# sara-nl/saraGAN

Measured on AMD Instinct MI355X. Metric: 3D volumes/sec/node (G+D step) at 128x128x32, higher is better.
Workload: dtype bf16

## Files before the change

### saragan_amd/csrc/common.h

```cpp
#pragma once
#include <hip/hip_runtime.h>
#include <stdint.h>
#include <mutex>
#include "../../include/saragan_hip.h"

typedef __bf16 bf16_t;
typedef float f32x4 __attribute__((ext_vector_type(4)));
typedef float f32x16 __attribute__((ext_vector_type(16)));
typedef __bf16 bf16x8 __attribute__((ext_vector_type(8)));
typedef __bf16 bf16x4 __attribute__((ext_vector_type(4)));
typedef short s16x4 __attribute__((ext_vector_type(4)));
typedef uint32_t u32x4 __attribute__((ext_vector_type(4)));

#define SG_STORE16_GUARD(v) asm volatile("s_nop 1" ::"v"(v))
typedef uint32_t u32x2 __attribute__((ext_vector_type(2)));

#define SG_LAUNCH_CHECK()                          \
  do {                                             \
    hipError_t e__ = hipGetLastError();            \
    if (e__ != hipSuccess) return (int)e__;        \
  } while (0)

static inline hipStream_t sg_st(sg_stream_t s) { return (hipStream_t)s; }

struct sg_config {
  int fwd_lds, fwd_tg;
  int fwd_v1, fwd_no_pw, fwd_no_dense;
  int fwd_no_v3, fwd_no_v3s, fwd_no_v4, fwd_no_v5, fwd_no_ksplit;
  int fwd3p_16;
  int fwd3s_16;
  int fwd_no_3p;
  int fwd3_gx, fwd3_no_lean;
  int fwd4_gx, fwd4_no_lean, fwd4_no_wres;
  int wgrad_v1, wgrad_no_v3, wgrad_no_lean;
  int wgrad_no_w16;
  int wgrad3l_min_cols;
  int wgrad3l_16;
  int wgrad3l_reuse;
  int wgrad_v1_blocks;
  int dbg_flags;
  int no_small;
  int deterministic;
  int gemm_ks_model;
  int gemm_k333_maxvox;
  int no_gemm;
};
const sg_config& sg_cfg();

bool sg_gemm_conv_eligible(const sg_conv_shape* s, sg_dtype dt);
size_t sg_gemm_conv_workspace(const sg_conv_shape* s, sg_dtype dt);
int sg_gemm_conv_fwd(const void* x, const void* wp, void* y, const sg_conv_shape* s, const float* bias, int act, float slope,
                     const uint32_t* mask_bits, float mask_slope, uint32_t* sign_out, void* workspace, size_t workspace_bytes,
                     hipStream_t st, bool* used);

bool sg_small_eligible(const sg_conv_shape* s);
bool sg_small_wgrad_eligible(const sg_conv_shape* s);
size_t sg_small_tail_bytes(const sg_conv_shape* s);
size_t sg_small_wgrad_workspace(const sg_conv_shape* s);
int sg_small_pack(const float* w, float coef, int flip, void* tail, const sg_conv_shape* s, sg_dtype dt, hipStream_t st);
int sg_small_fwd(const void* x, const void* tail, void* y, const sg_conv_shape* s, const float* bias, int act, float slope,
                 int pixel_norm, float eps, float* pn_scale, const uint32_t* mask_bits, float mask_slope, uint32_t* sign_out,
                 sg_dtype dt, hipStream_t st);
int sg_small_wgrad(const void* x, const void* dy, float* dw, float* dbias, float coef, void* workspace, size_t workspace_bytes,
                   const sg_conv_shape* s, sg_dtype dt, hipStream_t st);

#define SG_ALLOW_160K_LDS(kern)                                                                                  \
  do {                                                                                                           \
    static std::once_flag once__;                                                                                \
    static hipError_t err__ = hipSuccess;                                                                        \
    std::call_once(once__, [&] {                                                                                 \
      err__ = hipFuncSetAttribute((const void*)(kern), hipFuncAttributeMaxDynamicSharedMemorySize, 160 * 1024);  \
    });                                                                                                          \
    if (err__ != hipSuccess) return (int)err__;                                                                  \
  } while (0)
static inline size_t sg_esize(sg_dtype dt) { return dt == SG_BF16 ? 2 : 4; }
static inline bool sg_aligned16(const void* p) { return (((uintptr_t)p) & 15) == 0; }

__device__ __forceinline__ void philox4x32_10(uint32_t c0, uint32_t c1, uint32_t c2, uint32_t c3, uint32_t k0,
                                              uint32_t k1, uint32_t out[4]) {
#pragma unroll
  for (int rnd = 0; rnd < 10; ++rnd) {
    const uint32_t hi0 = __umulhi(0xD2511F53u, c0), lo0 = 0xD2511F53u * c0;
    const uint32_t hi1 = __umulhi(0xCD9E8D57u, c2), lo1 = 0xCD9E8D57u * c2;
    const uint32_t n0 = hi1 ^ c1 ^ k0, n1 = lo1, n2 = hi0 ^ c3 ^ k1, n3 = lo0;
    c0 = n0; c1 = n1; c2 = n2; c3 = n3;
    k0 += 0x9E3779B9u; k1 += 0xBB67AE85u;
  }
  out[0] = c0; out[1] = c1; out[2] = c2; out[3] = c3;
}

struct sg_fastdiv {
  uint32_t d, m;
};
static inline __host__ __device__ sg_fastdiv sg_make_fastdiv(uint32_t d) {
  sg_fastdiv f;
  f.d = d;
  f.m = d <= 1 ? 0u : (uint32_t)((0x100000000ull + d - 1) / d);
  return f;
}
__device__ __forceinline__ uint32_t sg_div(uint32_t x, sg_fastdiv f) {
  return f.d <= 1 ? x : __umulhi(x, f.m);
}

template <typename T>
struct sg_traits;
template <>
struct sg_traits<float> {
  static constexpr int CH = 8;
  __device__ static __forceinline__ float to_f(float v) { return v; }
  __device__ static __forceinline__ float from_f(float v) { return v; }
};
template <>
struct sg_traits<bf16_t> {
  static constexpr int CH = 16;
  __device__ static __forceinline__ float to_f(bf16_t v) { return (float)v; }
  __device__ static __forceinline__ bf16_t from_f(float v) { return (bf16_t)v; }
};

template <typename T>
__device__ __forceinline__ f32x16 sg_mfma_chunk(u32x4 a, u32x4 b, f32x16 c);
template <>
__device__ __forceinline__ f32x16 sg_mfma_chunk<bf16_t>(u32x4 a, u32x4 b, f32x16 c) {
// ... 200 lines not shown
```

### saragan_amd/csrc/prof.hip

```cpp
#include "prof.h"
#include <mutex>
#include <vector>
#include <string.h>
#include <stdlib.h>
#include <atomic>

namespace {
struct Rec { int kind; sg_conv_shape shape; int dtype; hipEvent_t e0, e1; bool ok; const char* name; };
std::mutex g_mu;
bool g_on = false;
bool g_filter = false;
int g_fkind = 0;
sg_conv_shape g_fshape;
std::vector<Rec> g_recs;
const char* kVersion = "saragan_hip 0.4 (gfx950)";
}

bool sg_prof_on() { return g_on; }
thread_local const char* sg_tls_kernel = "";

namespace {
std::atomic<const sg_config*> g_cfg{nullptr};
int env_int(const char* name, int dflt) {
  const char* v = getenv(name);
  return v && *v ? atoi(v) : dflt;
}
const sg_config* read_config() {
  sg_config* c = new sg_config;
  c->fwd_lds = env_int("SG_FWD_LDS", 80 * 1024);
  c->fwd_tg = env_int("SG_FWD_TG", 0);
  c->fwd_v1 = env_int("SG_FWD_V1", 0);
  c->fwd_no_pw = env_int("SG_FWD_NO_PW", 0);
  c->fwd_no_dense = env_int("SG_FWD_NO_DENSE", 0);
  c->fwd_no_v3 = env_int("SG_FWD_NO_V3", 0);
  c->fwd_no_v3s = env_int("SG_FWD_NO_V3S", 0);
  c->wgrad_no_lean = env_int("SG_WGRAD_NO_LEAN", 0);
  c->wgrad_no_w16 = env_int("SG_WGRAD_NO_W16", 0);
  c->wgrad3l_16 = env_int("SG_WGRAD3L_16", 0);
  c->wgrad3l_reuse = env_int("SG_WGRAD3L_REUSE", 1);
  c->wgrad3l_min_cols = env_int("SG_WGRAD3L_MIN_COLS", 0);
  c->wgrad_v1_blocks = env_int("SG_WGRAD_V1_BLOCKS", 0);
  c->fwd_no_v4 = env_int("SG_FWD_NO_V4", 0);
  c->fwd_no_v5 = env_int("SG_FWD_NO_V5", 0);
  c->fwd_no_ksplit = env_int("SG_FWD_NO_KSPLIT", 0);
  c->fwd_no_3p = env_int("SG_FWD_NO_3P", 0);
  c->fwd3p_16 = env_int("SG_FWD3P_16", 1);
  c->fwd3s_16 = env_int("SG_FWD3S_16", 1);
  c->fwd3_gx = env_int("SG_FWD3_GX", 0);
  c->fwd3_no_lean = env_int("SG_FWD3_NO_LEAN", 0);
  c->fwd4_gx = env_int("SG_FWD4_GX", 0);
  c->fwd4_no_lean = env_int("SG_FWD4_NO_LEAN", 0);
  c->fwd4_no_wres = env_int("SG_FWD4_NO_WRES", 0);
  c->wgrad_v1 = env_int("SG_WGRAD_V1", 0);
  c->wgrad_no_v3 = env_int("SG_WGRAD_NO_V3", 0);
  c->dbg_flags = env_int("SG_DBG_FLAGS", 0);
  c->no_small = env_int("SG_NO_SMALL", 0);
  c->deterministic = env_int("SG_DETERMINISTIC", 0);
  c->no_gemm = env_int("SG_NO_GEMM", 0);
  c->gemm_ks_model = env_int("SG_GEMM_KS_MODEL", 0);
  c->gemm_k333_maxvox = env_int("SG_GEMM_K333_MAXVOX", 8192);
  return c;
}
}

const sg_config& sg_cfg() {
  const sg_config* c = g_cfg.load(std::memory_order_acquire);
  if (c == nullptr) {
    std::lock_guard<std::mutex> lk(g_mu);
    c = g_cfg.load(std::memory_order_acquire);
    if (c == nullptr) {
      c = read_config();
      g_cfg.store(c, std::memory_order_release);
    }
  }
  return *c;
}

extern "C" int sg_config_reload(void) {
  std::lock_guard<std::mutex> lk(g_mu);
  g_cfg.store(read_config(), std::memory_order_release);
  return SG_OK;
}

void sg_prof_begin(int kind, const sg_conv_shape* s, sg_dtype dt, hipStream_t st, int* slot) {
  std::lock_guard<std::mutex> lk(g_mu);
  if (g_filter && (kind != g_fkind || memcmp(s, &g_fshape, sizeof(sg_conv_shape)) != 0)) { *slot = -1; return; }
  Rec r; r.kind = kind; r.shape = *s; r.dtype = (int)dt; r.ok = false; r.name = "";
  if (hipEventCreate(&r.e0) != hipSuccess) { *slot = -1; return; }
  if (hipEventCreate(&r.e1) != hipSuccess) { (void)hipEventDestroy(r.e0); *slot = -1; return; }
  (void)hipEventRecord(r.e0, st);
  g_recs.push_back(r);
  *slot = (int)g_recs.size() - 1;
}

void sg_prof_end(int slot, hipStream_t st) {
  std::lock_guard<std::mutex> lk(g_mu);
  bool ok = slot >= 0;
  int idx = ok ? slot : -1 - slot;
  if (idx < 0 || idx >= (int)g_recs.size()) return;
  (void)hipEventRecord(g_recs[idx].e1, st);
  g_recs[idx].ok = ok;
}

void sg_prof_name(int slot, const char* name) {
  std::lock_guard<std::mutex> lk(g_mu);
  if (slot >= 0 && slot < (int)g_recs.size()) g_recs[slot].name = name;
}

extern "C" const char* sg_version(void) { return kVersion; }

extern "C" const char* sg_error_string(int code) {
  switch (code) {
    case SG_OK: return "ok";
    case SG_EINVAL: return "invalid argument (shape, null pointer or unsupported combination)";
    case SG_EWORKSPACE: return "workspace too small";
    case SG_EALIGN: return "pointer not 16-byte aligned";
    case SG_EUNSUPPORTED: return "no kernel covers this request";
    default: break;
  }
  if (code > 0) return hipGetErrorString((hipError_t)code);
  return "unknown error";
}

extern "C" int sg_prof_enable(int on) {
// ... 51 lines not shown
```

### saragan_amd/csrc/wgrad.hip

```cpp
#include "common.h"
#include "prof.h"
#include <stdlib.h>
#include <type_traits>

struct WgradArgs {
  const void* x;
  const void* dy;
  float* dwt;
  sg_tile_geom g;
  sg_tile_geom gy;
  int cin, cout, taps, kh, kw, tap0, taps_blk;
  int ciT, coT;
  int rs;
  int xbytes, ybytes;
  int ntiles;
  sg_fastdiv fnp;
  int vec_x, vec_y;
  int plane_rows;
  float* dbias;
  int64_t slab, bslab;
  int nslab;
  int dbg_flags;
  unsigned long long* dbg;
  const uint32_t* dy_mask;
// ... 1546 lines not shown
  *used = false;
  const bool w16 = KD == 3 && KH == 3 && KW == 3 && s->w == 16 && (s->h % 8) == 0 && (s->d % 2) == 0 && !a.dy_mask &&
                   !sg_cfg().wgrad_no_lean && !sg_cfg().wgrad_no_w16;
  a.g = sg_make_geom(s, 256, true, 2, w16 ? 8 : 4);
  const sg_tile_geom& g = a.g;
  if (g.TW != (w16 ? 16 : 32) || g.TN != 1 || g.TD * g.TH * g.TW != 256) return SG_OK;
  if (g.HD != 2 && g.HD != 4) return SG_OK;
  if (g.TD != 2 || g.TH != (w16 ? 8 : 4)) return SG_OK;
  if (g.HH > 127 || g.HW > 127) return SG_OK;
  if ((s->cin % 8) || (s->cout % 8)) return SG_OK;
  if ((int64_t)g.TN * s->d * s->h * s->w * (int64_t)(s->cin > s->cout ? s->cin : s->cout) >= (1ll << 31)) return SG_OK;
  const int ncol = g.nTn * g.nTh * g.nTw;
  const int pairs = a.ciT * a.coT;
  int gx = (256 / pairs) / 8 * 8;
  if (gx < 8) gx = 8;
  while (gx > 8 && ncol < 2 * gx && (gx - 8) * pairs >= (w16 ? 128 : 64)) gx -= 8;
  const int min_cols = sg_cfg().wgrad3l_min_cols > 0 ? sg_cfg().wgrad3l_min_cols : 2;
  if (ncol < (2 * gx < min_cols ? 2 * gx : min_cols) || g.nTd < 2) return SG_OK;
  a.gy = a.g;
  a.ntiles = ncol * g.nTd;
  a.rs = 64;
  a.plane_rows = (g.HH * g.HW + 15) & ~15;
  if (a.plane_rows / 16 > 16) return SG_OK;
  a.xbytes = g.HD * a.plane_rows * 64;
  a.ybytes = 256 * 64;
  size_t lds = 2ull * (a.xbytes + a.ybytes);
  if (lds > 160 * 1024) return SG_OK;
  a.tap0 = 0; a.taps_blk = a.taps;
  a.nslab = 2 * gx;
  const bool lean = KD == 3 && KH == 3 && KW == 3 && g.HH == 6 && g.HW == 34 && g.HD == 4 && a.plane_rows == 208 &&
                    s->w % 32 == 0 && !sg_cfg().wgrad_no_lean && (!g.ups || ((s->d | s->h | s->w) & 1) == 0);
  const bool lean16 = w16 && g.HH == 10 && g.HW == 18 && g.HD == 4 && (!g.ups || ((s->d | s->h | s->w) & 1) == 0);
  if (w16 && !lean16) return SG_OK;
  if (lean16 || lean) a.nslab = gx;
  if (lean) lds += 12288;
  const bool m16 = sg_cfg().wgrad3l_16 != 0;
  const bool ru = sg_cfg().wgrad3l_reuse != 0;
#define SG_LAUNCH_WGRAD3L_1(UPS_, DYM_, TW_, M16_, RU_, NAME_)                                                        \
  do {                                                                                                               \
    auto kern = conv_wgrad3l_kernel<UPS_, DYM_, TW_, M16_, RU_>;                                                     \
    SG_ALLOW_160K_LDS(kern);                                                                                         \
    SG_KNAME(NAME_);                                                                                                 \
    hipLaunchKernelGGL(kern, dim3((unsigned)gx, (unsigned)pairs), dim3(512), lds, st, a);                            \
  } while (0)
#define SG_LAUNCH_WGRAD3L(UPS_, DYM_, TW_, NAME_)                                                                     \
  do {                                                                                                               \
    if (m16 && ru) SG_LAUNCH_WGRAD3L_1(UPS_, DYM_, TW_, true, true, NAME_);                                          \
    else if (m16) SG_LAUNCH_WGRAD3L_1(UPS_, DYM_, TW_, true, false, NAME_);                                          \
    else if (ru) SG_LAUNCH_WGRAD3L_1(UPS_, DYM_, TW_, false, true, NAME_);                                           \
    else SG_LAUNCH_WGRAD3L_1(UPS_, DYM_, TW_, false, false, NAME_);                                                  \
  } while (0)
  if (lean16) {
    lds = 2ull * (4 * 208 * 64 + 256 * 64) + 12288;
    if (g.ups) SG_LAUNCH_WGRAD3L(true, false, 16, "conv_wgrad3l<ups,w16>");
    else SG_LAUNCH_WGRAD3L(false, false, 16, "conv_wgrad3l<w16>");
  } else if (a.dy_mask) {
    if (!lean || g.ups || ((s->d | s->h | s->w) & 1)) return SG_OK;
    SG_LAUNCH_WGRAD3L(false, true, 32, "conv_wgrad3l<dy gather>");
  } else if (lean && g.ups) {
    SG_LAUNCH_WGRAD3L(true, false, 32, "conv_wgrad3l<ups>");
  } else if (lean) {
    SG_LAUNCH_WGRAD3L(false, false, 32, "conv_wgrad3l");
#undef SG_LAUNCH_WGRAD3L
#undef SG_LAUNCH_WGRAD3L_1
  } else {
    auto kern = conv_wgrad3_kernel<KD, KH, KW>;
    SG_ALLOW_160K_LDS(kern);
    SG_KNAME("conv_wgrad3<%d,%d,%d>", KD, KH, KW);
    hipLaunchKernelGGL(kern, dim3((unsigned)gx, (unsigned)pairs), dim3(512), lds, st, a);
  }
  SG_LAUNCH_CHECK();
  *used = true;
  return SG_OK;
}

struct WgradPlanesArgs {
  const void* x;
  const void* dy;
  float* dwt;
  float* dbias;
  int cin, cout, ciT, coT;
  int ntiles;
  int64_t slab, bslab;
};

template <int HW_>
__device__ __forceinline__ void conv_wgrad_planes_body(const WgradPlanesArgs& a) {
  extern __shared__ __attribute__((aligned(16))) char smem[];
  constexpr int H = HW_, W = HW_, P = 128 / (H * W), RP = (H + 2) * (W + 2);
  constexpr int XROWS = P * RP, NPX = (XROWS * 4 + 255) / 256, NPY = 2, PPT = NPX + NPY;
  constexpr int XB = NPX * 4096, YB = 128 * 64, BUF = XB + YB;
  constexpr uint32_t DEAD = 0x80000000u;
  const int tid = threadIdx.x, lane = tid & 63;
  const int wave = __builtin_amdgcn_readfirstlane(tid >> 6);
  const int ci_t = blockIdx.y / a.coT, co_t = blockIdx.y % a.coT;
  const int cin = a.cin, cout = a.cout;
  uint32_t vx[NPX], vy[NPY];
#pragma unroll
  for (int k = 0; k < NPX; ++k) {
    const int it = tid + 256 * k;
    const int row = it >> 2, sub = it & 3;
    const int p = row / RP, rr = row - p * RP;
    const int hh = rr / (W + 2), hw = rr - hh * (W + 2);
    const bool in = row < XROWS && hh >= 1 && hh <= H && hw >= 1 && hw <= W;
    vx[k] = in ? (uint32_t)((((p * H + hh - 1) * W + hw - 1) * cin + ci_t * 32 + sub * 8) * 2) : DEAD;
  }
#pragma unroll
  for (int k = 0; k < NPY; ++k) {
    const int it = tid + 256 * k;
    vy[k] = (uint32_t)(((it >> 2) * cout + co_t * 32 + (it & 3) * 8) * 2);
  }
  const __amdgpu_buffer_rsrc_t rx = __builtin_amdgcn_make_buffer_rsrc(const_cast<void*>(a.x), 0, (int)((int64_t)a.ntiles * 128 * cin * 2), 0x00020000);
  const __amdgpu_buffer_rsrc_t ry = __builtin_amdgcn_make_buffer_rsrc(const_cast<void*>(a.dy), 0, (int)((int64_t)a.ntiles * 128 * cout * 2), 0x00020000);
  auto stage = [&](int t, int b) __attribute__((always_inline)) {
    const bool ok = t < a.ntiles;
    const uint32_t sx = ok ? (uint32_t)t * (uint32_t)(128 * cin * 2) : 0u, sy = ok ? (uint32_t)t * (uint32_t)(128 * cout * 2) : 0u;
    char* xb = smem + b * BUF;
#pragma unroll
    for (int k = 0; k < NPX; ++k)
      __builtin_amdgcn_raw_ptr_buffer_load_lds(rx, (lds_ptr_t)(xb + (tid + 256 * k) * 16 - lane * 16), 16, ok ? vx[k] : DEAD, sx, 0, 0);
#pragma unroll
    for (int k = 0; k < NPY; ++k)
      __builtin_amdgcn_raw_ptr_buffer_load_lds(ry, (lds_ptr_t)(xb + XB + (tid + 256 * k) * 16 - lane * 16), 16, ok ? vy[k] : DEAD, sy, 0, 0);
  };
  const int i16 = lane & 15, q16 = lane >> 4;
  const int colb = (16 * (q16 & 1) + 4 * (i16 & 3)) * 2;
  const int kb = 8 * (q16 >> 1) + (i16 >> 2);
  int xr[2], yr[2];
#pragma unroll
  for (int j = 0; j < 2; ++j) {
    const int m = kb + 4 * j;
    xr[j] = ((m / W + (wave < 3 ? wave : 0)) * (W + 2) + m % W) * 64 + colb;
    yr[j] = XB + m * 64 + colb;
  }
  const bool ones = wave == 3 && a.dbias != nullptr && ci_t == 0;
  f32x16 acc[3];
#pragma unroll
  for (int j = 0; j < 3; ++j)
#pragma unroll
    for (int i = 0; i < 16; ++i) acc[j][i] = 0.f;
  const u32x4 one8 = {0x3F803F80u, 0x3F803F80u, 0x3F803F80u, 0x3F803F80u};

  typedef s16x4 __attribute__((address_space(3))) * lds_s16x4_p;
  const int t0 = blockIdx.x, G = gridDim.x;
  stage(t0, 0);
  stage(t0 + G, 1);
  int b = 0;
  for (int t = t0; t < a.ntiles; t += G) {
    const int b2 = b >= 1 ? b - 1 : 2;
    stage(t + 2 * G, b2);
    asm volatile("s_waitcnt vmcnt(%0)" ::"n"(2 * PPT) : "memory");
    __syncthreads();
    const char* base = smem + b * BUF;
    if (wave < 3 || ones) {
#pragma unroll
      for (int ks = 0; ks < 8; ++ks) {
        const int xoff = H == 8 ? ((ks >> 2) * RP + (ks & 3) * 2 * (W + 2)) * 64 : ks * RP * 64;
        const s16x4 b0 = __builtin_amdgcn_ds_read_tr16_b64_v4i16((lds_s16x4_p)(base + yr[0] + ks * 1024));
        const s16x4 b1 = __builtin_amdgcn_ds_read_tr16_b64_v4i16((lds_s16x4_p)(base + yr[1] + ks * 1024));
        u32x4 bf;
        bf[0] = __builtin_bit_cast(u32x2, b0)[0]; bf[1] = __builtin_bit_cast(u32x2, b0)[1];
        bf[2] = __builtin_bit_cast(u32x2, b1)[0]; bf[3] = __builtin_bit_cast(u32x2, b1)[1];
        if (wave < 3) {
#pragma unroll
          for (int kw = 0; kw < 3; ++kw) {
            const s16x4 a0 = __builtin_amdgcn_ds_read_tr16_b64_v4i16((lds_s16x4_p)(base + xr[0] + xoff + kw * 64));
            const s16x4 a1 = __builtin_amdgcn_ds_read_tr16_b64_v4i16((lds_s16x4_p)(base + xr[1] + xoff + kw * 64));
            u32x4 af;
            af[0] = __builtin_bit_cast(u32x2, a0)[0]; af[1] = __builtin_bit_cast(u32x2, a0)[1];
            af[2] = __builtin_bit_cast(u32x2, a1)[0]; af[3] = __builtin_bit_cast(u32x2, a1)[1];
            acc[kw] = __builtin_amdgcn_mfma_f32_32x32x16_bf16(__builtin_bit_cast(bf16x8, af), __builtin_bit_cast(bf16x8, bf), acc[kw], 0, 0, 0);
          }
        } else {
          acc[0] = __builtin_amdgcn_mfma_f32_32x32x16_bf16(__builtin_bit_cast(bf16x8, one8), __builtin_bit_cast(bf16x8, bf), acc[0], 0, 0, 0);
        }
      }
    }
    __syncthreads();
    b = b == 2 ? 0 : b + 1;
  }
  asm volatile("s_waitcnt vmcnt(0)" ::: "memory");
  const int r = lane & 31, hh = lane >> 5;
  const bool slab = a.slab != 0;
  if (wave < 3) {
#pragma unroll
    for (int kw = 0; kw < 3; ++kw) {
      float* dst = a.dwt + (int64_t)blockIdx.x * a.slab + ((((int64_t)(wave * 3 + kw) * a.ciT + ci_t) * a.coT + co_t) << 10);
#pragma unroll
      for (int i = 0; i < 16; ++i) {
        const int row = (i & 3) + 8 * (i >> 2) + 4 * hh;
        sg_wg_out(dst + row * 32 + r, acc[kw][i], slab);
      }
    }
  } else if (ones && hh == 0) {
    sg_wg_out(a.dbias + (int64_t)blockIdx.x * a.bslab + co_t * 32 + r, acc[0][0], slab);
  }
}

__global__ __launch_bounds__(256, 2) void conv_wgrad_planes8_kernel(WgradPlanesArgs a) { conv_wgrad_planes_body<8>(a); }
__global__ __launch_bounds__(256, 2) void conv_wgrad_planes4_kernel(WgradPlanesArgs a) { conv_wgrad_planes_body<4>(a); }

static bool wgrad_planes_eligible(const sg_conv_shape* s) {
  if (s->kd != 1 || s->kh != 3 || s->kw != 3 || s->upsample_in || s->h != s->w || (s->h != 4 && s->h != 8)) return false;
  if ((s->cin % 32) || (s->cout % 32)) return false;
  const int P = 128 / (s->h * s->w);
  const int64_t planes = (int64_t)s->n * s->d;
  if (planes % P) return false;
  const int64_t vox = planes * s->h * s->w;
  return vox * (s->cin > s->cout ? s->cin : s->cout) * 2 < (1ll << 31);
}

static int launch_wgrad_planes(WgradArgs& a, const sg_conv_shape* s, hipStream_t st, bool* used) {
  *used = false;
  if (!wgrad_planes_eligible(s)) return SG_OK;
  WgradPlanesArgs p;
  p.x = a.x; p.dy = a.dy; p.dwt = a.dwt; p.dbias = a.dbias; p.cin = s->cin; p.cout = s->cout; p.ciT = a.ciT; p.coT = a.coT;
  p.ntiles = (int)((int64_t)s->n * s->d * s->h * s->w / 128);
  p.slab = a.slab; p.bslab = a.bslab;
  const int pairs = a.ciT * a.coT;
  int gx = sg_cdiv(512, pairs);
  if (gx > 16) gx = 16;
  if (gx > p.ntiles) gx = p.ntiles;
  a.nslab = gx;
  if (s->h == 8) {
    auto kern = conv_wgrad_planes8_kernel;
    SG_ALLOW_160K_LDS(kern);
    SG_KNAME("conv_wgrad_planes<8>");
    constexpr int XB = ((2 * 100 * 4 + 255) / 256) * 4096;
    hipLaunchKernelGGL(kern, dim3((unsigned)gx, (unsigned)pairs), dim3(256), 3 * (size_t)(XB + 8192), st, p);
  } else {
    auto kern = conv_wgrad_planes4_kernel;
    SG_ALLOW_160K_LDS(kern);
    SG_KNAME("conv_wgrad_planes<4>");
    constexpr int XB = ((8 * 36 * 4 + 255) / 256) * 4096;
    hipLaunchKernelGGL(kern, dim3((unsigned)gx, (unsigned)pairs), dim3(256), 3 * (size_t)(XB + 8192), st, p);
  }
  SG_LAUNCH_CHECK();
  *used = true;
  return SG_OK;
}

static size_t wgrad_tile_bytes(const sg_conv_shape* s) {
  const size_t need = (size_t)(s->kd * s->kh * s->kw) * sg_cdiv(s->cin, 32) * sg_cdiv(s->cout, 32) * 4096;
  const bool pointwise = s->kd * s->kh * s->kw == 1 && (s->cin <= 4 || s->cout <= 4);
  const size_t pw = pointwise ? (size_t)PW_WGRAD_MAX_BLOCKS * 5 * (size_t)(s->cin > s->cout ? s->cin : s->cout) * sizeof(float) : 0;
  return ((need > pw ? need : pw) + 255) & ~(size_t)255;
}

extern "C" int sg_conv3d_wgrad(const void* x, const void* dy, float* dw, float coef, void* workspace,
                               size_t workspace_bytes, const sg_conv_shape* s, sg_dtype dt, sg_stream_t st) {
  return sg_conv3d_wgrad_bias(x, dy, dw, nullptr, coef, workspace, workspace_bytes, s, dt, st);
}

static int wgrad_bias_impl(const void* x, const void* dy, float* dw, float* dbias, float coef, void* workspace,
                           size_t workspace_bytes, const sg_conv_shape* s, sg_dtype dt, sg_stream_t st, void* pw_dx,
                           const float* pw_wmat, const void* dy_mask = nullptr, float dy_mask_slope = 0.f, float dy_gain = 1.f,
                           unsigned flags = 0) {
  const int accumulate = (flags & SG_WGRAD_ACCUMULATE) ? 1 : 0;
  const bool clean_ws = (flags & SG_WGRAD_CLEAN_WORKSPACE) != 0;
  if (!conv_shape_ok_w(s) || !x || !dy || !dw || !workspace) return SG_EINVAL;
  if (!sg_aligned16(x) || !sg_aligned16(dy) || !sg_aligned16(workspace)) return SG_EALIGN;
  if (dy_mask && (dt != SG_BF16 || s->kd != 3 || s->kh != 3 || s->kw != 3 || s->upsample_in || (s->cout % 32) ||
                  sg_cfg().wgrad_v1 || sg_cfg().wgrad_no_v3 || !sg_is_pow2f(dy_gain)))
    return SG_EUNSUPPORTED;
  const size_t need = sg_conv3d_wgrad_workspace(s, dt);
  if (workspace_bytes < need) return SG_EWORKSPACE;
  hipStream_t hs = sg_st(st);
  sg_prof_scope prof(1, s, dt, hs);
  {
    const int taps1 = s->kd * s->kh * s->kw;
    const int cs = s->cin < s->cout ? s->cin : s->cout, cb = s->cin < s->cout ? s->cout : s->cin;
    const int E = dt == SG_BF16 ? 8 : 4;
    if (taps1 == 1 && cs <= 4 && !s->upsample_in && cb % E == 0 && cb / E <= 256 && 256 % (cb / E) == 0) {
      if (accumulate || clean_ws) { prof.done(SG_EUNSUPPORTED); return SG_EUNSUPPORTED; }
      const int small_is_cin = s->cin <= s->cout ? 1 : 0;
      const void* sm = small_is_cin ? x : dy;
      const void* bg = small_is_cin ? dy : x;
      const int64_t nvox = (int64_t)s->n * s->d * s->h * s->w;
      const int rows = 256 / (cb / E);
      int64_t nb = (nvox + rows - 1) / rows;
      if (nb > PW_WGRAD_MAX_BLOCKS) nb = PW_WGRAD_MAX_BLOCKS;
      float* part = reinterpret_cast<float*>(workspace);
      const int ones = (dbias != nullptr && small_is_cin) ? 1 : 0;
      SG_KNAME("pw_wgrad_partial");
      if (pw_dx && (!small_is_cin || cb / E > 64)) { prof.done(SG_EUNSUPPORTED); return SG_EUNSUPPORTED; }
      if (dt == SG_BF16 && cs == 1)
        hipLaunchKernelGGL((pw_wgrad_partial_kernel<bf16_t, 1>), dim3((unsigned)nb), dim3(256), 0, hs, (const bf16_t*)sm,
                           (const bf16_t*)bg, part, nvox, cs, cb, ones, (bf16_t*)pw_dx, pw_wmat);
      else if (dt == SG_BF16)
        hipLaunchKernelGGL(pw_wgrad_partial_kernel<bf16_t>, dim3((unsigned)nb), dim3(256), 0, hs, (const bf16_t*)sm,
                           (const bf16_t*)bg, part, nvox, cs, cb, ones, (bf16_t*)pw_dx, pw_wmat);
      else
        hipLaunchKernelGGL(pw_wgrad_partial_kernel<float>, dim3((unsigned)nb), dim3(256), 0, hs, (const float*)sm,
                           (const float*)bg, part, nvox, cs, cb, ones, (float*)pw_dx, pw_wmat);
      hipLaunchKernelGGL(pw_wgrad_final_kernel, dim3((unsigned)(((cs + ones) * cb + 31) / 32)), dim3(256), 0, hs, part,
                         dw, coef, (int)nb, cs, cb, small_is_cin, ones ? dbias : nullptr);
      int e0 = (int)hipGetLastError();
      if (e0 == 0 && dbias && !ones)
        e0 = sg_bias_act_bwd(dy, nullptr, nullptr, dbias, reinterpret_cast<char*>(workspace) + wgrad_tile_bytes(s), nvox,
                             s->cout, 0.f, dt, st);
      prof.done(e0);
      return e0;
    }
  }
  if (pw_dx) { prof.done(SG_EUNSUPPORTED); return SG_EUNSUPPORTED; }
  if (sg_small_wgrad_eligible(s) && !sg_cfg().no_small) {
    if (accumulate || clean_ws) { prof.done(SG_EUNSUPPORTED); return SG_EUNSUPPORTED; }
    const int rc_s = sg_small_wgrad(x, dy, dw, dbias, coef, workspace, workspace_bytes, s, dt, hs);
    prof.done(rc_s);
    return rc_s;
  }
  const size_t tile_bytes = (size_t)(s->kd * s->kh * s->kw) * sg_cdiv(s->cin, 32) * sg_cdiv(s->cout, 32) * 4096;
  const bool det = sg_cfg().deterministic != 0;
  const size_t ns_max = det ? (size_t)wgrad_slab_count(s) : 1;
  hipError_t e = hipSuccess;
  const size_t tile_al = (tile_bytes + 255) & ~(size_t)255;
  float* bias_staged = (!det && dbias) ? reinterpret_cast<float*>(reinterpret_cast<char*>(workspace) + tile_al) : nullptr;
  if (bias_staged && tile_al + (size_t)s->cout * sizeof(float) > ns_max * wgrad_tile_bytes(s) + sg_bias_act_bwd_workspace(s->cout)) {
    prof.done(SG_EWORKSPACE);
    return SG_EWORKSPACE;
  }
  if (!det && !clean_ws)
    e = hipMemsetAsync(workspace, 0, bias_staged ? tile_al + (size_t)s->cout * sizeof(float) : tile_bytes, hs);
  if (e != hipSuccess) { prof.done((int)e); return (int)e; }
  WgradArgs a;
  a.dbias = bias_staged ? bias_staged : dbias;
  a.slab = det ? (int64_t)(wgrad_tile_bytes(s) / 4) : 0;
  a.bslab = det ? (int64_t)(wgrad_bias_slab_bytes(s) / 4) : 0;
  a.nslab = 1;
  float* bias_slabs = reinterpret_cast<float*>(reinterpret_cast<char*>(workspace) + ns_max * wgrad_tile_bytes(s) +
                                               sg_bias_act_bwd_workspace(s->cout));
  if (det && dbias) a.dbias = bias_slabs;
  bool db_done = false;
  a.dbg_flags = sg_cfg().dbg_flags;
  a.dbg = g_dbg_ts;
  a.x = x; a.dy = dy; a.dwt = reinterpret_cast<float*>(workspace);
  a.dy_mask = reinterpret_cast<const uint32_t*>(dy_mask); a.dy_mask_slope = dy_mask_slope; a.dy_gain = dy_gain;
  a.cin = s->cin; a.cout = s->cout;
  a.taps = s->kd * s->kh * s->kw; a.kh = s->kh; a.kw = s->kw;
  a.ciT = sg_cdiv(s->cin, 32); a.coT = sg_cdiv(s->cout, 32);
  int rc = SG_OK;
  bool used = false;
  if (dt == SG_BF16 && !sg_cfg().wgrad_v1 && !sg_cfg().wgrad_no_v3) {
    if (s->kd == 3 && s->kh == 3 && s->kw == 3) rc = launch_wgrad3<3, 3, 3>(a, s, hs, &used);
    db_done = used;
  }
  if (dy_mask && rc == SG_OK && !used) { prof.done(SG_EUNSUPPORTED); return SG_EUNSUPPORTED; }
  if (rc == SG_OK && !used && dt == SG_BF16 && !sg_cfg().wgrad_v1 && !sg_cfg().no_gemm)
  {
    rc = launch_wgrad_planes(a, s, hs, &used);
    if (used) db_done = true;
  }
  if (rc == SG_OK && !used && dt == SG_BF16 && !sg_cfg().wgrad_v1) {
    if (s->kd == 3 && s->kh == 3 && s->kw == 3) rc = launch_wgrad2<3, 3, 3>(a, s, hs, &used);
    else if (s->kd == 1 && s->kh == 3 && s->kw == 3) rc = launch_wgrad2<1, 3, 3>(a, s, hs, &used);
  }
  if (rc == SG_OK && used) {  }
  else if (rc != SG_OK) {  }
  else if (dt == SG_BF16) rc = launch_wgrad<bf16_t, 256>(a, s, hs);
  else if (dt == SG_F32) rc = launch_wgrad<float, 128>(a, s, hs);
  else rc = SG_EINVAL;
  if (rc == SG_OK) {
    const int64_t total = (int64_t)a.taps * s->cin * s->cout;
    int blocks = (int)((total + 255) / 256);
    if (blocks > 2048) blocks = 2048;
    hipLaunchKernelGGL(wgrad_finalize_kernel, dim3(blocks), dim3(256), 0, hs, a.dwt, dw, coef, a.taps, s->cin,
                       s->cout, a.ciT, a.coT, det ? a.nslab : 1, a.slab, (bias_staged && db_done) ? bias_staged : nullptr, dbias,
                       accumulate, (clean_ws && !det) ? 1 : 0);
    if (det && dbias && db_done)
      hipLaunchKernelGGL(wgrad_bias_slabs_kernel, dim3((unsigned)sg_cdiv(s->cout, 256)), dim3(256), 0, hs, bias_slabs, dbias, s->cout,
                         a.nslab, a.bslab);
    hipError_t e2 = hipGetLastError();
    if (e2 != hipSuccess) rc = (int)e2;
  }
  if (rc == SG_OK && dbias && !db_done)
    rc = sg_bias_act_bwd(dy, nullptr, nullptr, dbias,
                         reinterpret_cast<char*>(workspace) + ns_max * wgrad_tile_bytes(s) + (clean_ws ? wgrad_bias_slab_bytes(s) : 0),
                         (int64_t)s->n * s->d * s->h * s->w, s->cout, 0.f, dt, st);
  prof.done(rc);
  return rc;
}

extern "C" int sg_conv3d_wgrad_bias(const void* x, const void* dy, float* dw, float* dbias, float coef, void* workspace,
                                    size_t workspace_bytes, const sg_conv_shape* s, sg_dtype dt, sg_stream_t st) {
  return wgrad_bias_impl(x, dy, dw, dbias, coef, workspace, workspace_bytes, s, dt, st, nullptr, nullptr);
}

extern "C" int sg_conv3d_wgrad_bias_up_masked(const void* x, const void* dy_half, const void* mask_bits, float mask_slope, float dy_gain,
                                              float* dw, float* dbias, float coef, void* workspace, size_t workspace_bytes,
                                              const sg_conv_shape* s, sg_dtype dt, sg_stream_t st) {
  if (!mask_bits) return SG_EINVAL;
  if (!sg_aligned16(mask_bits)) return SG_EALIGN;
  return wgrad_bias_impl(x, dy_half, dw, dbias, coef, workspace, workspace_bytes, s, dt, st, nullptr, nullptr, mask_bits, mask_slope, dy_gain);
}
// ... 25 lines not shown
```

Measured before the change: 630.0.

## Add whole-K weight-gradient kernels that write dW directly, skipping split-K reduction

Adds a whole-K variant of the planes weight-gradient kernel. Each block owns one (cin,cout) tile pair and loops over all spatial tiles with a 5-deep LDS ring and a software-pipelined MFMA k-loop. It writes coef-scaled dW directly, with optional accumulate, instead of a zeroed workspace, atomics and a reduction pass. It also adds an upsample-gather form and a separate outer-product kernel for 1x1x1 convs with at most 128 voxels. These aim to remove the memset and reduction launches and contention for small-spatial, wide-channel layers. The cost is one block per CU with K work done serially, which may underuse the GPU if the number of tile pairs is small.

```diff
diff --git a/saragan_amd/csrc/common.h b/saragan_amd/csrc/common.h
--- a/saragan_amd/csrc/common.h
+++ b/saragan_amd/csrc/common.h
@@ -38,6 +38,7 @@
   int wgrad3l_16;
   int wgrad3l_reuse;
   int wgrad_v1_blocks;
+  int wgrad_wholek;
   int dbg_flags;
   int no_small;
   int deterministic;
diff --git a/saragan_amd/csrc/prof.hip b/saragan_amd/csrc/prof.hip
--- a/saragan_amd/csrc/prof.hip
+++ b/saragan_amd/csrc/prof.hip
@@ -40,6 +40,7 @@
   c->wgrad3l_reuse = env_int("SG_WGRAD3L_REUSE", 1);
   c->wgrad3l_min_cols = env_int("SG_WGRAD3L_MIN_COLS", 0);
   c->wgrad_v1_blocks = env_int("SG_WGRAD_V1_BLOCKS", 0);
+  c->wgrad_wholek = env_int("SG_WGRAD_WHOLEK", 1);
   c->fwd_no_v4 = env_int("SG_FWD_NO_V4", 0);
   c->fwd_no_v5 = env_int("SG_FWD_NO_V5", 0);
   c->fwd_no_ksplit = env_int("SG_FWD_NO_KSPLIT", 0);
diff --git a/saragan_amd/csrc/wgrad.hip b/saragan_amd/csrc/wgrad.hip
--- a/saragan_amd/csrc/wgrad.hip
+++ b/saragan_amd/csrc/wgrad.hip
@@ -1652,10 +1652,66 @@
   int cin, cout, ciT, coT;
   int ntiles;
   int64_t slab, bslab;
+  float* dw;
+  float coef;
+  int accumulate;
 };
 
-template <int HW_>
+template <int HW_, bool XS>
+struct sg_planes_kloop {
+  static constexpr int W = HW_, RP = (W + 2) * (W + 2);
+  struct Frag { s16x4 b0, b1, a0[3], a1[3]; };
+  template <int KS>
+  static __device__ __forceinline__ void load(int ya, int xa0, int xa1, Frag& f) {
+    constexpr int xoff = HW_ == 8 ? ((KS >> 2) * RP + (KS & 3) * 2 * (W + 2)) * 64 : KS * RP * 64;
+    asm volatile("ds_read_b64_tr_b16 %0, %1 offset:%2" : "=v"(f.b0) : "v"(ya), "n"(KS * 1024));
+    asm volatile("ds_read_b64_tr_b16 %0, %1 offset:%2" : "=v"(f.b1) : "v"(ya), "n"(KS * 1024 + 256));
+    if constexpr (XS) {
+      asm volatile("ds_read_b64_tr_b16 %0, %1 offset:%2" : "=v"(f.a0[0]) : "v"(xa0), "n"(xoff));
+      asm volatile("ds_read_b64_tr_b16 %0, %1 offset:%2" : "=v"(f.a1[0]) : "v"(xa1), "n"(xoff));
+      asm volatile("ds_read_b64_tr_b16 %0, %1 offset:%2" : "=v"(f.a0[1]) : "v"(xa0), "n"(xoff + 64));
+      asm volatile("ds_read_b64_tr_b16 %0, %1 offset:%2" : "=v"(f.a1[1]) : "v"(xa1), "n"(xoff + 64));
+      asm volatile("ds_read_b64_tr_b16 %0, %1 offset:%2" : "=v"(f.a0[2]) : "v"(xa0), "n"(xoff + 128));
+      asm volatile("ds_read_b64_tr_b16 %0, %1 offset:%2" : "=v"(f.a1[2]) : "v"(xa1), "n"(xoff + 128));
+    }
+  }
+  template <int KS>
+  static __device__ __forceinline__ void step(int ya, int xa0, int xa1, f32x16 (&acc)[3], Frag (&f)[2]) {
+    if constexpr (KS < 8) {
+      if constexpr (KS + 1 < 8) load<KS + 1>(ya, xa0, xa1, f[(KS + 1) & 1]);
+      asm volatile("s_waitcnt lgkmcnt(%0)" ::"n"(KS + 1 < 8 ? (XS ? 8 : 2) : 0));
+      __builtin_amdgcn_sched_barrier(0);
+      const Frag& c = f[KS & 1];
+      u32x4 bf;
+      bf[0] = __builtin_bit_cast(u32x2, c.b0)[0]; bf[1] = __builtin_bit_cast(u32x2, c.b0)[1];
+      bf[2] = __builtin_bit_cast(u32x2, c.b1)[0]; bf[3] = __builtin_bit_cast(u32x2, c.b1)[1];
+      if constexpr (XS) {
+#pragma unroll
+        for (int kw = 0; kw < 3; ++kw) {
+          u32x4 af;
+          af[0] = __builtin_bit_cast(u32x2, c.a0[kw])[0]; af[1] = __builtin_bit_cast(u32x2, c.a0[kw])[1];
+          af[2] = __builtin_bit_cast(u32x2, c.a1[kw])[0]; af[3] = __builtin_bit_cast(u32x2, c.a1[kw])[1];
+          acc[kw] = __builtin_amdgcn_mfma_f32_32x32x16_bf16(__builtin_bit_cast(bf16x8, af), __builtin_bit_cast(bf16x8, bf), acc[kw], 0, 0, 0);
+        }
+      } else {
+        const u32x4 one8 = {0x3F803F80u, 0x3F803F80u, 0x3F803F80u, 0x3F803F80u};
+        acc[0] = __builtin_amdgcn_mfma_f32_32x32x16_bf16(__builtin_bit_cast(bf16x8, one8), __builtin_bit_cast(bf16x8, bf), acc[0], 0, 0, 0);
+      }
+      __builtin_amdgcn_sched_barrier(0);
+      step<KS + 1>(ya, xa0, xa1, acc, f);
+    }
+  }
+  static __device__ __forceinline__ void run(int ya, int xa0, int xa1, f32x16 (&acc)[3]) {
+    Frag f[2];
+    load<0>(ya, xa0, xa1, f[0]);
+    step<0>(ya, xa0, xa1, acc, f);
+  }
+};
+
+template <int HW_, bool WK = false, bool UPS = false>
 __device__ __forceinline__ void conv_wgrad_planes_body(const WgradPlanesArgs& a) {
+  static_assert(WK || !UPS, "the gather exists in the whole-K form only");
+  constexpr int NB = WK ? 5 : 3;
   extern __shared__ __attribute__((aligned(16))) char smem[];
   constexpr int H = HW_, W = HW_, P = 128 / (H * W), RP = (H + 2) * (W + 2);
   constexpr int XROWS = P * RP, NPX = (XROWS * 4 + 255) / 256, NPY = 2, PPT = NPX + NPY;
@@ -1663,7 +1719,8 @@
   constexpr uint32_t DEAD = 0x80000000u;
   const int tid = threadIdx.x, lane = tid & 63;
   const int wave = __builtin_amdgcn_readfirstlane(tid >> 6);
-  const int ci_t = blockIdx.y / a.coT, co_t = blockIdx.y % a.coT;
+  const int pair = WK ? blockIdx.x : blockIdx.y;
+  const int ci_t = pair / a.coT, co_t = pair % a.coT;
   const int cin = a.cin, cout = a.cout;
   uint32_t vx[NPX], vy[NPY];
 #pragma unroll
@@ -1673,18 +1730,22 @@
     const int p = row / RP, rr = row - p * RP;
     const int hh = rr / (W + 2), hw = rr - hh * (W + 2);
     const bool in = row < XROWS && hh >= 1 && hh <= H && hw >= 1 && hw <= W;
-    vx[k] = in ? (uint32_t)((((p * H + hh - 1) * W + hw - 1) * cin + ci_t * 32 + sub * 8) * 2) : DEAD;
-  }
+    if constexpr (UPS)
+      vx[k] = in ? (uint32_t)(((((p >> 1) * (H / 2) + ((hh - 1) >> 1)) * (W / 2) + ((hw - 1) >> 1)) * cin + ci_t * 32 + sub * 8) * 2) : DEAD;
+    else
+      vx[k] = in ? (uint32_t)((((p * H + hh - 1) * W + hw - 1) * cin + ci_t * 32 + sub * 8) * 2) : DEAD;
+  }
+  constexpr int XVOX = UPS ? 16 : 128;
 #pragma unroll
   for (int k = 0; k < NPY; ++k) {
     const int it = tid + 256 * k;
     vy[k] = (uint32_t)(((it >> 2) * cout + co_t * 32 + (it & 3) * 8) * 2);
   }
-  const __amdgpu_buffer_rsrc_t rx = __builtin_amdgcn_make_buffer_rsrc(const_cast<void*>(a.x), 0, (int)((int64_t)a.ntiles * 128 * cin * 2), 0x00020000);
+  const __amdgpu_buffer_rsrc_t rx = __builtin_amdgcn_make_buffer_rsrc(const_cast<void*>(a.x), 0, (int)((int64_t)a.ntiles * XVOX * cin * 2), 0x00020000);
   const __amdgpu_buffer_rsrc_t ry = __builtin_amdgcn_make_buffer_rsrc(const_cast<void*>(a.dy), 0, (int)((int64_t)a.ntiles * 128 * cout * 2), 0x00020000);
   auto stage = [&](int t, int b) __attribute__((always_inline)) {
     const bool ok = t < a.ntiles;
-    const uint32_t sx = ok ? (uint32_t)t * (uint32_t)(128 * cin * 2) : 0u, sy = ok ? (uint32_t)t * (uint32_t)(128 * cout * 2) : 0u;
+    const uint32_t sx = ok ? (uint32_t)t * (uint32_t)(XVOX * cin * 2) : 0u, sy = ok ? (uint32_t)t * (uint32_t)(128 * cout * 2) : 0u;
     char* xb = smem + b * BUF;
 #pragma unroll
     for (int k = 0; k < NPX; ++k)
@@ -1712,17 +1773,24 @@
   const u32x4 one8 = {0x3F803F80u, 0x3F803F80u, 0x3F803F80u, 0x3F803F80u};
 
   typedef s16x4 __attribute__((address_space(3))) * lds_s16x4_p;
-  const int t0 = blockIdx.x, G = gridDim.x;
-  stage(t0, 0);
-  stage(t0 + G, 1);
+  auto ring_barrier = [&]() __attribute__((always_inline)) {
+    if constexpr (WK) asm volatile("s_waitcnt lgkmcnt(0)\n\ts_barrier" ::: "memory");
+    else __syncthreads();
+  };
+  const int t0 = WK ? 0 : (int)blockIdx.x, G = WK ? 1 : (int)gridDim.x;
+#pragma unroll
+  for (int i = 0; i < NB - 1; ++i) stage(t0 + i * G, i);
   int b = 0;
   for (int t = t0; t < a.ntiles; t += G) {
-    const int b2 = b >= 1 ? b - 1 : 2;
-    stage(t + 2 * G, b2);
-    asm volatile("s_waitcnt vmcnt(%0)" ::"n"(2 * PPT) : "memory");
-    __syncthreads();
+    const int b2 = b >= 1 ? b - 1 : NB - 1;
+    stage(t + (NB - 1) * G, b2);
+    asm volatile("s_waitcnt vmcnt(%0)" ::"n"((NB - 1) * PPT) : "memory");
+    ring_barrier();
     const char* base = smem + b * BUF;
-    if (wave < 3 || ones) {
+    if constexpr (WK) {
+      if (wave < 3) sg_planes_kloop<HW_, true>::run(b * BUF + yr[0], b * BUF + xr[0], b * BUF + xr[1], acc);
+      else if (ones) sg_planes_kloop<HW_, false>::run(b * BUF + yr[0], 0, 0, acc);
+    } else if (wave < 3 || ones) {
 #pragma unroll
       for (int ks = 0; ks < 8; ++ks) {
         const int xoff = H == 8 ? ((ks >> 2) * RP + (ks & 3) * 2 * (W + 2)) * 64 : ks * RP * 64;
@@ -1746,11 +1814,28 @@
         }
       }
     }
-    __syncthreads();
-    b = b == 2 ? 0 : b + 1;
+    ring_barrier();
+    b = b == NB - 1 ? 0 : b + 1;
   }
   asm volatile("s_waitcnt vmcnt(0)" ::: "memory");
   const int r = lane & 31, hh = lane >> 5;
+  if constexpr (WK) {
+    if (wave < 3) {
+#pragma unroll
+      for (int kw = 0; kw < 3; ++kw) {
+        float* dst = a.dw + ((int64_t)(wave * 3 + kw) * cin + ci_t * 32) * cout + co_t * 32 + r;
+#pragma unroll
+        for (int i = 0; i < 16; ++i) {
+          float* q = dst + (int64_t)((i & 3) + 8 * (i >> 2) + 4 * hh) * cout;
+          const float v = __fmul_rn(a.coef, acc[kw][i]);
+          *q = a.accumulate ? __fadd_rn(*q, v) : v;
+        }
+      }
+    } else if (ones && hh == 0) {
+      a.dbias[co_t * 32 + r] = acc[0][0];
+    }
+    return;
+  }
   const bool slab = a.slab != 0;
   if (wave < 3) {
 #pragma unroll
@@ -1769,6 +1854,10 @@
 
 __global__ __launch_bounds__(256, 2) void conv_wgrad_planes8_kernel(WgradPlanesArgs a) { conv_wgrad_planes_body<8>(a); }
 __global__ __launch_bounds__(256, 2) void conv_wgrad_planes4_kernel(WgradPlanesArgs a) { conv_wgrad_planes_body<4>(a); }
+__global__ __launch_bounds__(256) void conv_wgrad_planes8_wholek_kernel(WgradPlanesArgs a) { conv_wgrad_planes_body<8, true>(a); }
+__global__ __launch_bounds__(256) void conv_wgrad_planes4_wholek_kernel(WgradPlanesArgs a) { conv_wgrad_planes_body<4, true>(a); }
+__global__ __launch_bounds__(256) void conv_wgrad_planes8_wholek_ups_kernel(WgradPlanesArgs a) { conv_wgrad_planes_body<8, true, true>(a); }
+__global__ __launch_bounds__(256) void conv_wgrad_planes4_wholek_ups_kernel(WgradPlanesArgs a) { conv_wgrad_planes_body<4, true, true>(a); }
 
 static bool wgrad_planes_eligible(const sg_conv_shape* s) {
   if (s->kd != 1 || s->kh != 3 || s->kw != 3 || s->upsample_in || s->h != s->w || (s->h != 4 && s->h != 8)) return false;
@@ -1807,6 +1896,135 @@
   }
   SG_LAUNCH_CHECK();
   *used = true;
+  return SG_OK;
+}
+
+static constexpr int WGRAD_WHOLEK_MAX_TILES = 48;
+static bool wgrad_planes_wholek_eligible(const sg_conv_shape* s) {
+  sg_conv_shape t = *s;
+  t.upsample_in = 0;
+  if (!wgrad_planes_eligible(&t) || sg_cdiv(s->cin, 32) * sg_cdiv(s->cout, 32) < 256) return false;
+  return s->upsample_in || (int64_t)s->n * s->d * s->h * s->w / 128 <= WGRAD_WHOLEK_MAX_TILES;
+}
+
+static int launch_wgrad_planes_wholek(const void* x, const void* dy, float* dw, float* dbias, float coef, int accumulate,
+                                      const sg_conv_shape* s, hipStream_t st) {
+  WgradPlanesArgs p;
+  p.x = x; p.dy = dy; p.dwt = nullptr; p.dbias = dbias; p.cin = s->cin; p.cout = s->cout;
+  p.ciT = s->cin / 32; p.coT = s->cout / 32;
+  p.ntiles = (int)((int64_t)s->n * s->d * s->h * s->w / 128);
+  p.slab = p.bslab = 0;
+  p.dw = dw; p.coef = coef; p.accumulate = accumulate;
+  const unsigned pairs = (unsigned)(p.ciT * p.coT);
+  constexpr size_t LDS8 = 5 * (size_t)(((2 * 100 * 4 + 255) / 256) * 4096 + 8192), LDS4 = 5 * (size_t)(((8 * 36 * 4 + 255) / 256) * 4096 + 8192);
+  static_assert(LDS8 > 80 * 1024 && LDS4 <= 160 * 1024, "one block per CU, within the LDS");
+#define SG_LAUNCH_PLANES_WK(KERN_, NAME_, LDS_)                                      \
+  do {                                                                               \
+    auto kern = KERN_;                                                               \
+    SG_ALLOW_160K_LDS(kern);                                                         \
+    SG_KNAME(NAME_);                                                                 \
+    hipLaunchKernelGGL(kern, dim3(pairs), dim3(256), LDS_, st, p);                   \
+  } while (0)
+  if (s->h == 8 && !s->upsample_in) SG_LAUNCH_PLANES_WK(conv_wgrad_planes8_wholek_kernel, "conv_wgrad_planes<8,whole K>", LDS8);
+  else if (s->h == 8) SG_LAUNCH_PLANES_WK(conv_wgrad_planes8_wholek_ups_kernel, "conv_wgrad_planes<8,whole K,ups>", LDS8);
+  else if (!s->upsample_in) SG_LAUNCH_PLANES_WK(conv_wgrad_planes4_wholek_kernel, "conv_wgrad_planes<4,whole K>", LDS4);
+  else SG_LAUNCH_PLANES_WK(conv_wgrad_planes4_wholek_ups_kernel, "conv_wgrad_planes<4,whole K,ups>", LDS4);
+#undef SG_LAUNCH_PLANES_WK
+  SG_LAUNCH_CHECK();
+  return SG_OK;
+}
+
+struct WgradOuterArgs {
+  const void* x;
+  const void* dy;
+  float* dw;
+  float* dbias;
+  int cin, cout, coT, coG, K;
+  float coef;
+  int accumulate;
+};
+
+__global__ __launch_bounds__(256) void conv_wgrad_outer_kernel(WgradOuterArgs a) {
+  extern __shared__ __attribute__((aligned(16))) char smem[];
+  constexpr int TB = 128 * 64;
+  constexpr uint32_t DEAD = 0x80000000u;
+  const int tid = threadIdx.x, lane = tid & 63;
+  const int wave = __builtin_amdgcn_readfirstlane(tid >> 6);
+  const int ci_t = blockIdx.x / a.coG, co_t0 = (blockIdx.x % a.coG) * 4;
+  const int cin = a.cin, cout = a.cout;
+  const int ksteps = (a.K + 15) >> 4, kp = ksteps * 16;
+  const __amdgpu_buffer_rsrc_t rx = __builtin_amdgcn_make_buffer_rsrc(const_cast<void*>(a.x), 0, a.K * cin * 2, 0x00020000);
+  const __amdgpu_buffer_rsrc_t ry = __builtin_amdgcn_make_buffer_rsrc(const_cast<void*>(a.dy), 0, a.K * cout * 2, 0x00020000);
+#pragma unroll
+  for (int k = 0; k < 2; ++k) {
+    if (64 * k < kp) {
+      const int it = tid + 256 * k, row = it >> 2, sub = it & 3;
+      __builtin_amdgcn_raw_ptr_buffer_load_lds(rx, (lds_ptr_t)(smem + it * 16 - lane * 16), 16, (uint32_t)((row * cin + ci_t * 32 + sub * 8) * 2), 0, 0, 0);
+    }
+  }
+#pragma unroll
+  for (int k = 0; k < 8; ++k) {
+    if (64 * (k & 1) < kp) {
+      const int it = tid + 256 * k, row = (it >> 2) & 127, sub = it & 3, co_t = co_t0 + (k >> 1);
+      __builtin_amdgcn_raw_ptr_buffer_load_lds(ry, (lds_ptr_t)(smem + TB + it * 16 - lane * 16), 16,
+                                               co_t < a.coT ? (uint32_t)((row * cout + co_t * 32 + sub * 8) * 2) : DEAD, 0, 0, 0);
+    }
+  }
+  asm volatile("s_waitcnt vmcnt(0)" ::: "memory");
+  __syncthreads();
+  const int co_t = co_t0 + wave;
+  if (co_t >= a.coT) return;
+  const int i16 = lane & 15, q16 = lane >> 4;
+  const int colb = (16 * (q16 & 1) + 4 * (i16 & 3)) * 2;
+  const int kb = 8 * (q16 >> 1) + (i16 >> 2);
+  const bool ones = a.dbias != nullptr && ci_t == 0;
+  const u32x4 one8 = {0x3F803F80u, 0x3F803F80u, 0x3F803F80u, 0x3F803F80u};
+  f32x16 acc, accb;
+#pragma unroll
+  for (int i = 0; i < 16; ++i) acc[i] = accb[i] = 0.f;
+  typedef s16x4 __attribute__((address_space(3))) * lds_s16x4_p;
+  const char* xb = smem + kb * 64 + colb;
+  const char* yb = smem + TB + wave * TB + kb * 64 + colb;
+  for (int ks = 0; ks < ksteps; ++ks) {
+    const s16x4 a0 = __builtin_amdgcn_ds_read_tr16_b64_v4i16((lds_s16x4_p)(xb + ks * 1024));
+    const s16x4 a1 = __builtin_amdgcn_ds_read_tr16_b64_v4i16((lds_s16x4_p)(xb + ks * 1024 + 256));
+    const s16x4 b0 = __builtin_amdgcn_ds_read_tr16_b64_v4i16((lds_s16x4_p)(yb + ks * 1024));
+    const s16x4 b1 = __builtin_amdgcn_ds_read_tr16_b64_v4i16((lds_s16x4_p)(yb + ks * 1024 + 256));
+    u32x4 af, bf;
+    af[0] = __builtin_bit_cast(u32x2, a0)[0]; af[1] = __builtin_bit_cast(u32x2, a0)[1];
+    af[2] = __builtin_bit_cast(u32x2, a1)[0]; af[3] = __builtin_bit_cast(u32x2, a1)[1];
+    bf[0] = __builtin_bit_cast(u32x2, b0)[0]; bf[1] = __builtin_bit_cast(u32x2, b0)[1];
+    bf[2] = __builtin_bit_cast(u32x2, b1)[0]; bf[3] = __builtin_bit_cast(u32x2, b1)[1];
+    acc = __builtin_amdgcn_mfma_f32_32x32x16_bf16(__builtin_bit_cast(bf16x8, af), __builtin_bit_cast(bf16x8, bf), acc, 0, 0, 0);
+    if (ones) accb = __builtin_amdgcn_mfma_f32_32x32x16_bf16(__builtin_bit_cast(bf16x8, one8), __builtin_bit_cast(bf16x8, bf), accb, 0, 0, 0);
+  }
+  const int r = lane & 31, hh = lane >> 5;
+  float* dst = a.dw + (int64_t)ci_t * 32 * cout + co_t * 32 + r;
+#pragma unroll
+  for (int i = 0; i < 16; ++i) {
+    float* q = dst + (int64_t)((i & 3) + 8 * (i >> 2) + 4 * hh) * cout;
+    const float v = __fmul_rn(a.coef, acc[i]);
+    *q = a.accumulate ? __fadd_rn(*q, v) : v;
+  }
+  if (ones && hh == 0) a.dbias[co_t * 32 + r] = accb[0];
+}
+
+static bool wgrad_outer_eligible(const sg_conv_shape* s) {
+  if (s->kd * s->kh * s->kw != 1 || s->upsample_in || (s->cin % 32) || (s->cout % 32)) return false;
+  if ((int64_t)s->n * s->d * s->h * s->w > 128) return false;
+  if (s->cin > (1 << 22) || s->cout > (1 << 22)) return false;
+  return (int64_t)(s->cin / 32) * (s->cout / 32) >= 256;
+}
+
+static int launch_wgrad_outer(const void* x, const void* dy, float* dw, float* dbias, float coef, int accumulate,
+                              const sg_conv_shape* s, hipStream_t st) {
+  WgradOuterArgs p;
+  p.x = x; p.dy = dy; p.dw = dw; p.dbias = dbias; p.cin = s->cin; p.cout = s->cout;
+  p.coT = s->cout / 32; p.coG = sg_cdiv(p.coT, 4); p.K = s->n * s->d * s->h * s->w;
+  p.coef = coef; p.accumulate = accumulate;
+  SG_KNAME("conv_wgrad_outer");
+  hipLaunchKernelGGL(conv_wgrad_outer_kernel, dim3((unsigned)((s->cin / 32) * p.coG)), dim3(256), 5 * 128 * 64, st, p);
+  SG_LAUNCH_CHECK();
   return SG_OK;
 }
 
@@ -1880,6 +2098,15 @@
     prof.done(rc_s);
     return rc_s;
   }
+  if (dt == SG_BF16 && sg_cfg().wgrad_wholek && !sg_cfg().wgrad_v1 && !sg_cfg().no_gemm && !dy_mask) {
+    const bool planes = wgrad_planes_wholek_eligible(s);
+    if (planes || wgrad_outer_eligible(s)) {
+      const int rc_w = planes ? launch_wgrad_planes_wholek(x, dy, dw, dbias, coef, accumulate, s, hs)
+                              : launch_wgrad_outer(x, dy, dw, dbias, coef, accumulate, s, hs);
+      prof.done(rc_w);
+      return rc_w;
+    }
+  }
   const size_t tile_bytes = (size_t)(s->kd * s->kh * s->kw) * sg_cdiv(s->cin, 32) * sg_cdiv(s->cout, 32) * 4096;
   const bool det = sg_cfg().deterministic != 0;
   const size_t ns_max = det ? (size_t)wgrad_slab_count(s) : 1;
```

Result: no change. 634.8 (median of 6 runs) (+0.8%).
